# notu97/GS-SLAM-Analytica_Jacobian

Hardware: AMD Instinct MI355X
Metric: Gaussian-pixel interactions/sec (fwd+Jacobian), 640x480 (higher is better)
Workload: dtype f32; 1 GPU; cfg2: 50000 Gaussians (SH degree 3, 16 coeffs), 640x480; one step = one mapping window of 8 keyframes with distinct cameras: forward splat + analytical-Jacobian backward (dL/dmu, dL/dSigma->conic, per-Gaussian grads summed over the window, one dL/dtau per keyframe)

## Files before the change

### gs-slam-analytica_jacobian_amd/csrc/gsaj_common.h

```cpp
#pragma once
#include <hip/hip_runtime.h>
#include <stddef.h>
#include <stdint.h>

#include "../../include/gsaj.h"

#define GSAJ_WAVE 64
#define TILE GSAJ_TILE
#define TILE_PIXELS (TILE * TILE)
#define PRE_BLOCK 256
#define GB_BLOCK 64
#define REC_F4 3
#define IGRAD_F 12


#include "workspace.h"
#define WS_MEMBER(field, type, count) type *field;
#define WS_TAKE(field, type, count) w->field = c.take<type>(count);
#define WS_SHIFT(field, type, count) w.field = gsaj_shift(w.field, off);

#define GEOM_WS_FIELDS(X)                                                                                                          \
  X(depths, float, P)                               \
  X(cov3D, float, P * 6)               \
  X(clamped, uint8_t, P * 3)                                                                                                       \
  X(tiles_touched, uint32_t, P)                                                                                                    \
  X(point_offsets, uint32_t, P)     \
  X(internal_radii, int, P)                                                                                                        \
  X(block_sums, uint32_t, nblk)                               \
  X(tau_partials, float, ((P + 31) / 32 + 1) * 8)    \
  X(splat, float4, P * 3)                     \
  X(splat16, float4, P * 2)        \
                                          \
  X(scat, uint2, P)                        \
                                                                                                           \
  X(gsum, float4, P * 3)               \
struct GeomWS { GEOM_WS_FIELDS(WS_MEMBER) };

static inline size_t geom_carve(Carver c, size_t P, GeomWS *w) {
  size_t nblk = (P + PRE_BLOCK - 1) / PRE_BLOCK;
  if (nblk == 0) nblk = 1;
  GEOM_WS_FIELDS(WS_TAKE)
  return c.used();
}

#define TILE_REP 1
#define LDS_TILES_MAX 8192
#define SORT_CAP 16384
#define N_COUNTERS 64
#define ERR_PREFILTERED 1u
#define ERR_INTERNAL 2u
#define ERR_CAPACITY 4u
#define ERR_TILE_LIST 8u

#define IMAGE_WS_HEAD(X)                                                                                                           \
  X(final_T, float, N)                                                                                                             \
  X(n_contrib, uint32_t, N)                                                                                                        \
  X(ranges, uint2, tiles)
#define IMAGE_WS_ZEROED(X)                                                                                                         \
  X(counters, uint32_t, N_COUNTERS)                                                                                                \
  X(tile_count, uint32_t, tiles * TILE_REP)                                                                                        \
  X(tile_cursor, uint32_t, tiles * TILE_REP)
#define IMAGE_WS_TAIL(X)                                                                                                           \
  X(tile_offset, uint32_t, tiles * TILE_REP + 1)                                    \
  X(sticky, uint32_t, 16)             \
                                                                                                \
  X(tile_order, uint32_t, tiles)
#define IMAGE_WS_FIELDS(X) IMAGE_WS_HEAD(X) IMAGE_WS_ZEROED(X) IMAGE_WS_TAIL(X)
struct ImageWS {
  IMAGE_WS_FIELDS(WS_MEMBER)
  size_t zero_bytes;
};

static inline size_t image_carve(Carver c, int W, int H, ImageWS *w) {
  const size_t N = (size_t)W * H;
  const size_t tiles = (size_t)((W + TILE - 1) / TILE) * ((H + TILE - 1) / TILE);
  IMAGE_WS_HEAD(WS_TAKE)
  const size_t z0 = c.used();
  IMAGE_WS_ZEROED(WS_TAKE)
  w->zero_bytes = c.used() - z0;
  IMAGE_WS_TAIL(WS_TAKE)
  return c.used();
}

#define BIN_WS_FIELDS(X)                                                                                                           \
  X(keys_unsorted, uint64_t, R)      \
  X(keys, uint64_t, R)              \
                                       \
                                                                                                    \
  X(point_list, uint32_t, R)           \
                                                                                                              \
  X(inst_grad, float4, R * REC_F4)                        \
  X(reached, uint8_t, R)            \
                                                          \
  X(taken, uint32_t, R)            \
                                    \
                                       \
struct BinWS { BIN_WS_FIELDS(WS_MEMBER) };

static inline size_t bin_carve(Carver c, size_t R, BinWS *w) {
  if (R == 0) R = 1;
  BIN_WS_FIELDS(WS_TAKE)
  return c.used();
}

struct ViewStrides {
  size_t geom, image, bin;
};
#ifdef __HIPCC__
#include <type_traits>
template <typename T>
__device__ __forceinline__ T *gsaj_shift(T *p, size_t bytes) {
  typedef typename std::conditional<std::is_const<T>::value, const char, char>::type byte_t;
  return reinterpret_cast<T *>(reinterpret_cast<byte_t *>(p) + bytes);
}
__device__ __forceinline__ GeomWS geom_view(GeomWS w, size_t off) {
  GEOM_WS_FIELDS(WS_SHIFT)
  return w;
}
__device__ __forceinline__ ImageWS image_view(ImageWS w, size_t off) {
  IMAGE_WS_FIELDS(WS_SHIFT)
  return w;
}
#endif

struct Carved { GeomWS g; BinWS b; ImageWS im; ViewStrides vs; };

void gsaj_set_error(const char *fmt, ...);
#define GSAJ_HIP_CHECK(expr)                                                          \
  do {                                                                                \
    hipError_t _e = (expr);                                                           \
    if (_e != hipSuccess) {                                                           \
      gsaj_set_error("%s failed: %s (%s:%d)", #expr, hipGetErrorString(_e), __FILE__, __LINE__); \
      return GSAJ_ERR_HIP;                                                            \
    }                                                                                 \
  } while (0)

enum GsajStage {
  ST_PREPROCESS = 0, ST_SCAN, ST_EMIT_KEYS, ST_SORT, ST_RANGES_RECORDS, ST_RENDER_FWD, ST_RENDER_BWD, ST_GAUSSIAN_BWD,
  ST_TAU_FINALIZE, ST_DENSE_BWD, ST_DENSE_REDUCE, ST_SCATTER, ST_TILE_SORT, ST_GATHER_SUMS, ST_COUNT
};
void gsaj_prof_mark(int stage, int is_stop, hipStream_t s);
struct GsajProfScope {
  int stage;
  hipStream_t s;
  GsajProfScope(int st, hipStream_t stream) : stage(st), s(stream) { gsaj_prof_mark(stage, 0, s); }
  ~GsajProfScope() { gsaj_prof_mark(stage, 1, s); }
};

struct FwdParams {
  int P, D, M, W, H;
  const float *means3D, *shs, *colors_precomp, *opacities, *scales, *rotations, *cov3D_precomp;
  const float *viewmatrix, *projmatrix, *campos;
  float scale_modifier, tanfovx, tanfovy, focal_x, focal_y;
  int prefiltered;
  int grid_x, grid_y;
  int capacity;
  int sort_cap;
  int bpw;
  int views;
};

struct PreprocessPlan {
  int bpw;
  int workgroups;
  bool hist_lds;
};
struct ScatterPlan {
  int gpt;
  int workgroups;
  bool counters_lds;
};
PreprocessPlan plan_preprocess(int P, int views, int grid_x, int grid_y);
ScatterPlan plan_scatter(int P, int views, int grid_x, int grid_y);

#define LDS_DEFAULT_LIMIT 65536
struct LdsRequest {
  size_t dynamic_bytes, static_bytes, limit_bytes;
  int variant;
};
constexpr size_t lds_static_round(size_t bytes) { return (bytes + 3) / 4 * 4; }
LdsRequest lds_preprocess(const PreprocessPlan &pl, int grid_x, int grid_y, bool sh16);
LdsRequest lds_frame_scan(const PreprocessPlan &pl, int grid_x, int grid_y);
LdsRequest lds_scatter(const ScatterPlan &pl, int grid_x, int grid_y);
struct SortPlan {
  int launches;
  int keys[2];
  int pass[2];
  LdsRequest lds[2];
};
SortPlan plan_tile_sort(int sort_cap);
LdsRequest lds_gaussian_bwd(int M, bool has_shs);
bool lds_stereo_winner(int W, int D, LdsRequest *out);

int launch_preprocess(const FwdParams &p, int *radii, int *n_touched, const GeomWS &g, const ImageWS &im, ViewStrides vs,
                      hipStream_t s);
int launch_tile_binning(int P, int sort_cap, int rec16, int grid_x, int grid_y, const GeomWS &g, const BinWS &b, const ImageWS &im,
                        int views, ViewStrides vs, hipStream_t s);
struct FusedLoss;
int launch_render_forward(int P, int W, int H, int grid_x, int grid_y, const float *bg, const GeomWS &g, const BinWS &b,
                          const ImageWS &im, float *out_color, float *out_depth, float *out_opacity, int *n_touched, int views,
                          ViewStrides vs, hipStream_t s, const FusedLoss *fl = nullptr);
int gsaj_fwd_loss_slots(int W, int H);
int launch_loss_finalize(const FusedLoss &fl, int nslots, int W, int H, const uint32_t *aborted, float *out_scalars, hipStream_t s,
                         int views = 1, size_t abort_stride = 0, float *out_dexposure = nullptr);
int launch_render_backward(int R, int W, int H, int grid_x, int grid_y, const float *bg, const GeomWS &g, const BinWS &b,
                           const ImageWS &im, const float *dL_dpix, const float *dL_dpix_depth, int views, ViewStrides vs,
                           hipStream_t s, const FusedLoss *fl = nullptr);
int launch_export_taken(int W, int H, int grid_x, int grid_y, const BinWS &b, const ImageWS &im, uint32_t *out, hipStream_t s);
struct BwdParams {
  int P, D, M, W, H;
  const float *means3D, *shs, *scales, *rotations, *cov3Ds;
  const float *viewmatrix, *projmatrix, *projmatrix_raw, *campos;
  float scale_modifier, tanfovx, tanfovy, focal_x, focal_y;
  int grid_x, grid_y;
  const int *radii;
  float *dL_dmean2D, *dL_dconic, *dL_dopacity, *dL_dcolor, *dL_ddepth, *dL_dmean3D, *dL_dcov3D, *dL_dsh, *dL_dscale,
      *dL_drot, *dL_dtau, *dL_dtau_sum;
};
int launch_gaussian_backward(const BwdParams &p, const GeomWS &g, const BinWS &b, const ImageWS &im, hipStream_t s);
int launch_gather_sums(int P, int K, const int *radii, const GeomWS &g, const BinWS &b, const ImageWS &im, ViewStrides vs, hipStream_t s);
int launch_gaussian_backward_batch(const BwdParams &p, int K, const GeomWS &g, const BinWS &b, const ImageWS &im, ViewStrides vs,
                                   int accumulate, int gather, hipStream_t s);
size_t gsaj_jac_rows_bytes(int P);
int gsaj_jac_slots(int W, int H);
int launch_splat_jac(const BwdParams &p, int K, const GeomWS &g, const ImageWS &im, float *rows, ViewStrides vs, size_t rows_stride,
                     hipStream_t s);
struct JacOut {
  float *jac;
  float *color, *depth;
  const float *seed_c, *seed_d;
  const float *curv_c, *curv_d;
  float *partials;
  float delta;
};
int launch_render_jac(const BwdParams &p, int K, const float *bg, const Carved &c, const float *rows, size_t rows_stride, const JacOut &jo,
                      const FusedLoss *fl, int joint, hipStream_t s);
int launch_gn_reduce(const float *partials, int n, const ImageWS &im, float *H_out, float *g_out, hipStream_t s);
int launch_mark_visible(int P, const float *means3D, const float *viewmatrix, uint8_t *present, hipStream_t s);
void launch_exclusive_scan_u32(int n, uint32_t *v, hipStream_t s);
int launch_select_rank_f32(int W, int H, const float *values, uint32_t rank, uint32_t *out_key, void *seed_ws, hipStream_t s);
hipError_t launch_stereo_paths(int D, int W, int H, int first_col, int P1, int P2, int paths, const uint16_t *C, uint32_t *S, hipStream_t s);

#ifdef __HIPCC__
__device__ __forceinline__ float3 xform4x3(const float *m, float3 p) {
  return make_float3(m[0] * p.x + m[4] * p.y + m[8] * p.z + m[12], m[1] * p.x + m[5] * p.y + m[9] * p.z + m[13],
                     m[2] * p.x + m[6] * p.y + m[10] * p.z + m[14]);
}
__device__ __forceinline__ float4 xform4x4(const float *m, float3 p) {
  return make_float4(m[0] * p.x + m[4] * p.y + m[8] * p.z + m[12], m[1] * p.x + m[5] * p.y + m[9] * p.z + m[13],
                     m[2] * p.x + m[6] * p.y + m[10] * p.z + m[14], m[3] * p.x + m[7] * p.y + m[11] * p.z + m[15]);
}
__device__ __forceinline__ float ndc2pix(float v, int S) { return (float)((((double)v + 1.0) * (double)S - 1.0) * 0.5); }

__device__ __forceinline__ uint32_t gsaj_tile_band(const uint32_t *__restrict__ sticky) {
  const uint32_t band = sticky[1];
  return sticky[2] == ~band ? band : 0u;
}
__device__ __forceinline__ void tile_rect(float px, float py, int r, int gx, int gy, uint32_t band, int &x0, int &y0, int &x1,
                                          int &y1) {
  const int ylo = band ? (int)(band & 0xffffu) : 0, yhi = band ? min(gy, (int)(band >> 16)) : gy;
  x0 = min(gx, max(0, (int)((px - (float)r) / (float)TILE)));
  y0 = min(yhi, max(ylo, (int)((py - (float)r) / (float)TILE)));
  x1 = min(gx, max(0, (int)((px + (float)r + (float)(TILE - 1)) / (float)TILE)));
  y1 = min(yhi, max(ylo, (int)((py + (float)r + (float)(TILE - 1)) / (float)TILE)));
}
#define GSAJ_LOG2E 1.4426950408889634f
__device__ __forceinline__ float3 gsaj_prescale_conic(float a, float b, float c) {
  return make_float3((-0.5f * GSAJ_LOG2E) * a, -GSAJ_LOG2E * b, (-0.5f * GSAJ_LOG2E) * c);
}
__device__ __forceinline__ float gsaj_power2(float dx, float dy, float kx, float ky, float kz) {
  const float t = ky * dy;
  const float u = kz * dy;
  return __builtin_fmaf(dx, __builtin_fmaf(kx, dx, t), u * dy);
}
__device__ __forceinline__ bool quadrant_relevant(float mx, float my, float a, float b, float c, float o, float X0,
                                                  float Y0) {
  const float dxl = mx - (X0 + 7.0f), dxh = mx - X0;
  const float dyl = my - (Y0 + 7.0f), dyh = my - Y0;
  const bool pd = a > 0.f && c > 0.f && (a * c - b * b) > 0.f;
  const bool inside = dxl <= 0.f && dxh >= 0.f && dyl <= 0.f && dyh >= 0.f;
  const float ic = __builtin_amdgcn_rcpf(c), ia = __builtin_amdgcn_rcpf(a);
  float q = 3.0e38f;
  {
    const float y0 = fminf(fmaxf(-b * dxl * ic, dyl), dyh);
    q = fminf(q, a * dxl * dxl + 2.f * b * dxl * y0 + c * y0 * y0);
    const float y1 = fminf(fmaxf(-b * dxh * ic, dyl), dyh);
    q = fminf(q, a * dxh * dxh + 2.f * b * dxh * y1 + c * y1 * y1);
    const float x0 = fminf(fmaxf(-b * dyl * ia, dxl), dxh);
    q = fminf(q, a * x0 * x0 + 2.f * b * x0 * dyl + c * dyl * dyl);
    const float x1 = fminf(fmaxf(-b * dyh * ia, dxl), dxh);
    q = fminf(q, a * x1 * x1 + 2.f * b * x1 * dyh + c * dyh * dyh);
  }
  const float qs = fmaxf(q * 0.999f - 1.0e-3f, 0.f);
  const bool reach = o * __expf(-0.5f * qs) >= (0.99f / 255.0f);
  return !pd || inside || reach;
}
__device__ __forceinline__ float3 cross3(float3 a, float3 b) {
  return make_float3(a.y * b.z - a.z * b.y, a.z * b.x - a.x * b.z, a.x * b.y - a.y * b.x);
}
#endif

#define REC16_F4 2
#ifdef __HIPCC__
#include <hip/hip_fp16.h>
__device__ __forceinline__ uint32_t gsaj_pack_h2(float a, float b) {
  const __half2 h = __floats2half2_rn(a, b);
  return *reinterpret_cast<const uint32_t *>(&h);
}
__device__ __forceinline__ float2 gsaj_unpack_h2(uint32_t u) { return __half22float2(*reinterpret_cast<const __half2 *>(&u)); }
__device__ __forceinline__ void gsaj_load_row(const float4 *__restrict__ splat, const float4 *__restrict__ splat16, uint32_t id,
                                              bool rec16, float4 &q0, float4 &q1, float4 &q2) {
  if (!rec16) {
    const float4 *s = splat + (size_t)id * REC_F4;
    const float4 r0 = s[0], r1 = s[1], r2 = s[2];
    q0 = make_float4(r0.x, r0.y, r2.w, r0.w);
    q1 = r1;
    q2 = make_float4(r2.x, r2.y, r2.z, r0.z);
    return;
  }
  const float4 *s = splat16 + (size_t)id * REC16_F4;
  const float4 p0 = s[0], p1 = s[1];
  const float2 ab = gsaj_unpack_h2(__float_as_uint(p1.x)), co = gsaj_unpack_h2(__float_as_uint(p1.y));
  const float2 rg = gsaj_unpack_h2(__float_as_uint(p1.z)), bz = gsaj_unpack_h2(__float_as_uint(p1.w));
  q0 = p0;
  q1 = make_float4(ab.x, ab.y, co.x, co.y);
  q2 = make_float4(rg.x, rg.y, bz.x, 0.f);
}
#endif

#ifdef __HIPCC__
__device__ __forceinline__ float4 gsaj_load_f4_unaligned(const void *src) {
  typedef float f4u __attribute__((ext_vector_type(4), aligned(4)));
  const f4u v = *reinterpret_cast<const __attribute__((address_space(1))) f4u *>((unsigned long long)src);
  return make_float4(v.x, v.y, v.z, v.w);
}
__device__ __forceinline__ uint32_t gsaj_load_u32_global(const uint32_t *src) {
  return *reinterpret_cast<const __attribute__((address_space(1))) uint32_t *>((unsigned long long)src);
}
__device__ __forceinline__ uint2 gsaj_load_u64_device(const uint2 *src) {
  const unsigned long long v = __hip_atomic_load(reinterpret_cast<const __attribute__((address_space(1))) unsigned long long *>((unsigned long long)src),
                                                 __ATOMIC_RELAXED, __HIP_MEMORY_SCOPE_AGENT);
  return make_uint2((uint32_t)v, (uint32_t)(v >> 32));
}
#endif

#ifdef GSAJ_BLOCK_TRACE
#define GSAJ_TRACE_MAX 65536
#define GSAJ_TRACE_DEFINE(NAME)                                                                               \
  __device__ unsigned long long g_trace_##NAME[4 * GSAJ_TRACE_MAX];                                           \
  extern "C" int gsaj_trace_read_##NAME(unsigned long long *host, int nwaves) {                               \
    return (int)hipMemcpyFromSymbol(host, HIP_SYMBOL(g_trace_##NAME), sizeof(unsigned long long) * 4 * nwaves); \
  }
#define GSAJ_TRACE_BEGIN(NAME)                                                                                \
  {                                                                                                           \
    const unsigned tw_ = (blockIdx.y * gridDim.x + blockIdx.x) * (blockDim.x >> 6) + (threadIdx.x >> 6);      \
    if ((threadIdx.x & 63) == 0 && tw_ < GSAJ_TRACE_MAX) {                                                    \
      g_trace_##NAME[4 * tw_ + 0] = wall_clock64();                                                           \
      g_trace_##NAME[4 * tw_ + 2] = __builtin_amdgcn_s_getreg((4) | (0 << 6) | (31 << 11));                   \
      g_trace_##NAME[4 * tw_ + 3] = __builtin_amdgcn_s_getreg((20) | (0 << 6) | (31 << 11));                  \
    }                                                                                                         \
  }
#define GSAJ_TRACE_END(NAME)                                                                                  \
  {                                                                                                           \
    const unsigned tw_ = (blockIdx.y * gridDim.x + blockIdx.x) * (blockDim.x >> 6) + (threadIdx.x >> 6);      \
    if ((threadIdx.x & 63) == 0 && tw_ < GSAJ_TRACE_MAX) g_trace_##NAME[4 * tw_ + 1] = wall_clock64();        \
  }
#else
#define GSAJ_TRACE_DEFINE(NAME)
#define GSAJ_TRACE_BEGIN(NAME)
#define GSAJ_TRACE_END(NAME)
#endif
```

### gs-slam-analytica_jacobian_amd/csrc/render_fwd.hip

```cpp
#include "gsaj_common.h"
#include "loss_terms.h"
#include "wave_reduce.h"

#define FWD_CHUNK 64
#define FWD_PAD 8
#define FWD_PAIR_F4 6
typedef float v2f __attribute__((ext_vector_type(2)));

#ifndef GSAJ_FWD_THREADS
#define GSAJ_FWD_THREADS 64
#endif
#define FWD_WAVES (GSAJ_FWD_THREADS / 64)

GSAJ_TRACE_DEFINE(fwd)

template <bool LOSS>
__global__ __launch_bounds__(GSAJ_FWD_THREADS) __attribute__((amdgpu_waves_per_eu(6, 8))) void k_render_fwd(int W, int H, int gx, int tiles, int P, ImageWS im,
                                                    const float4 *__restrict__ splat, const float4 *__restrict__ splat16,
                                                    const float *__restrict__ bg,
                                                    float *__restrict__ out_color, float *__restrict__ out_depth,
                                                    float *__restrict__ out_opacity, int *__restrict__ n_touched,
                                                    const uint32_t *__restrict__ point_list, uint32_t *__restrict__ taken,
                                                    ViewStrides vs, FusedLoss fl) {
  {
    const size_t view = blockIdx.y, HWv = (size_t)H * W;
    im = image_view(im, view * vs.image);
    splat = gsaj_shift(splat, view * vs.geom);
    splat16 = gsaj_shift(splat16, view * vs.geom);
    point_list = gsaj_shift(point_list, view * vs.bin);
    taken = gsaj_shift(taken, view * vs.bin);
    out_color += view * 3 * HWv;
    out_depth += view * HWv;
    out_opacity += view * HWv;
    n_touched += view * (size_t)P;
    if (LOSS) fused_loss_view(fl, view, HWv, gridDim.x);
  }
  const uint2 *__restrict__ ranges = im.ranges;
  float *__restrict__ final_T = im.final_T;
  uint32_t *__restrict__ n_contrib = im.n_contrib;
  uint32_t *__restrict__ counters = im.counters;
  __shared__ float4 rec_all[FWD_WAVES * ((FWD_CHUNK + FWD_PAD) / 2) * FWD_PAIR_F4];
  if (counters[4]) return;
  GSAJ_TRACE_BEGIN(fwd)
  const int tid = threadIdx.x, lane = tid & 63;
#if FWD_WAVES == 1
  const int wave = ((int)blockIdx.x >> 3) & 3;
  const int rank = ((int)blockIdx.x >> 5) * 8 + ((int)blockIdx.x & 7);
  if (rank >= tiles) {
    if (LOSS && lane == 0) reinterpret_cast<float4 *>(fl.partials)[blockIdx.x] = make_float4(0.f, 0.f, 0.f, 0.f);
    return;
  }
  const int tile = (int)min(im.tile_order[rank], (uint32_t)(tiles - 1));
  float4 *rec = rec_all;
#else
  const int wave = tid >> 6;
  const int tile = (int)min(im.tile_order[blockIdx.x], (uint32_t)(tiles - 1));
  float4 *rec = rec_all + wave * ((FWD_CHUNK + FWD_PAD) / 2) * FWD_PAIR_F4;
#endif
  const int ty = tile / gx, tx = tile - ty * gx;
  const int px = tx * TILE + (wave & 1) * 8 + (lane & 7);
  const int py = ty * TILE + (wave >> 1) * 8 + (lane >> 3);
  const bool inside = px < W && py < H;
  const float pxf = (float)px, pyf = (float)py;
  const float qx0 = (float)(tx * TILE + (wave & 1) * 8), qy0 = (float)(ty * TILE + (wave >> 1) * 8);
  const uint2 range = ranges[tile];

  unsigned long long done_m = __builtin_amdgcn_ballot_w64(!inside);
  float T = 1.0f;
  uint32_t last = 0;
  bool counting = true;

  auto sel = [](unsigned long long m, float a, float b) -> float {
    float r;
    asm("v_cndmask_b32_e64 %0, %1, %2, %3" : "=v"(r) : "v"(b), "v"(a), "s"(m));
    return r;
  };
  auto sel0 = [](unsigned long long m, float a) -> float {
    float r;
    asm("v_cndmask_b32_e64 %0, 0, %1, %2" : "=v"(r) : "v"(a), "s"(m));
    return r;
  };
  v2f Crg = {0.f, 0.f}, Cbd = {0.f, 0.f};
  const v2f px2 = {pxf, pxf}, py2 = {pyf, pyf};
  auto composite2 = [&](const float4 p0, const float4 p1, const float4 p2, const float4 cA, const float4 cB, const float2 pos,
                        float &T_afterA, unsigned long long &okA, unsigned long long &okB) {
    const v2f dx = v2f{p0.x, p0.y} - px2, dy = v2f{p0.z, p0.w} - py2;
    const v2f t = v2f{p1.z, p1.w} * dy;
    const v2f u = v2f{p2.x, p2.y} * dy;
    const v2f pw = __builtin_elementwise_fma(dx, __builtin_elementwise_fma(v2f{p1.x, p1.y}, dx, t), u * dy);
    const v2f oe = v2f{p2.z, p2.w} * v2f{__builtin_amdgcn_exp2f(pw.x), __builtin_amdgcn_exp2f(pw.y)};
    {
      const float alpha0 = fminf(0.99f, oe.x);
      const float tA = __builtin_fmaf(-alpha0, T, T);
      const unsigned long long pre = __builtin_amdgcn_ballot_w64(pw.x <= 0.0f) & __builtin_amdgcn_ballot_w64(alpha0 >= (1.0f / 255.0f)) & ~done_m;
      const unsigned long long sat = pre & __builtin_amdgcn_ballot_w64(tA < 0.0001f);
      done_m |= sat;
      okA = pre & ~sat;
      const float w = sel0(okA, alpha0 * T);
      const v2f w2 = {w, w};
      Crg = __builtin_elementwise_fma(v2f{cA.x, cA.y}, w2, Crg);
      Cbd = __builtin_elementwise_fma(v2f{cA.z, cA.w}, w2, Cbd);
      T = sel(okA, tA, T);
      last = __float_as_uint(sel(okA, pos.x, __uint_as_float(last)));
      T_afterA = T;
    }
    {
      const float alpha0 = fminf(0.99f, oe.y);
      const float tB = __builtin_fmaf(-alpha0, T, T);
      const unsigned long long pre = __builtin_amdgcn_ballot_w64(pw.y <= 0.0f) & __builtin_amdgcn_ballot_w64(alpha0 >= (1.0f / 255.0f)) & ~done_m;
      const unsigned long long sat = pre & __builtin_amdgcn_ballot_w64(tB < 0.0001f);
      done_m |= sat;
      okB = pre & ~sat;
      const float w = sel0(okB, alpha0 * T);
      const v2f w2 = {w, w};
      Crg = __builtin_elementwise_fma(v2f{cB.x, cB.y}, w2, Crg);
      Cbd = __builtin_elementwise_fma(v2f{cB.z, cB.w}, w2, Cbd);
      T = sel(okB, tB, T);
      last = __float_as_uint(sel(okB, pos.y, __uint_as_float(last)));
    }
  };

  if (~done_m != 0ull && range.x < range.y) {
    float4 q0, q1, q2;
    uint32_t id_cur = 0u, id_nxt = 0u;
    const bool rec16 = counters[7] != 0u;
    auto fetch_id = [&](uint32_t base) {
      if (base + (uint32_t)lane < range.y) id_nxt = point_list[base + lane];
    };
    auto fetch_row = [&](uint32_t base) {
      id_cur = id_nxt;
      if (base + (uint32_t)lane < range.y) gsaj_load_row(splat, splat16, id_nxt, rec16, q0, q1, q2);
    };
    float *recf = reinterpret_cast<float *>(rec);
    for (int i = lane; i < ((FWD_CHUNK + FWD_PAD) / 2) * FWD_PAIR_F4; i += 64) rec[i] = make_float4(0.f, 0.f, 0.f, 0.f);
    auto put = [&](int s, float x, float y, float kx, float ky, float kz, float o, float4 c, uint32_t pos, uint32_t id) {
      const int h = s & 1, pb = (s >> 1) * FWD_PAIR_F4;
      float *f = recf + pb * 4 + h;
      f[0] = x; f[2] = y; f[4] = kx; f[6] = ky; f[8] = kz; f[10] = o;
      rec[pb + 3 + h] = c;
      f[20] = __uint_as_float(pos); f[22] = __uint_as_float(id);
    };
    fetch_id(range.x);
    fetch_row(range.x);
    fetch_id(range.x + FWD_CHUNK);
    for (uint32_t base = range.x; base < range.y; base += FWD_CHUNK) {
      const int m = min((uint32_t)FWD_CHUNK, range.y - base);
      bool rel = false;
      const uint32_t id_here = id_cur;
      if (lane < m) rel = quadrant_relevant(q0.x, q0.y, q1.x, q1.y, q1.z, q1.w, qx0, qy0);
      const unsigned long long todo = __builtin_amdgcn_ballot_w64(rel);
      const int nrel = __popcll(todo);
      __builtin_amdgcn_wave_barrier();
      if (rel) {
        const int slot = __builtin_amdgcn_mbcnt_hi((uint32_t)(todo >> 32), __builtin_amdgcn_mbcnt_lo((uint32_t)todo, 0u));
        const float3 k = gsaj_prescale_conic(q1.x, q1.y, q1.z);
        put(slot, q0.x, q0.y, k.x, k.y, k.z, q1.w, make_float4(q2.x, q2.y, q2.z, q0.z), base - range.x + (uint32_t)lane + 1u, id_here);
      }
      if (lane < FWD_PAD) recf[((nrel + lane) >> 1) * FWD_PAIR_F4 * 4 + 10 + ((nrel + lane) & 1)] = 0.f;
      fetch_row(base + FWD_CHUNK);
      fetch_id(base + 2 * FWD_CHUNK);
      __builtin_amdgcn_fence(__ATOMIC_RELEASE, "wavefront");
      __builtin_amdgcn_wave_barrier();
      __builtin_amdgcn_fence(__ATOMIC_ACQUIRE, "wavefront");
      uint32_t cnt4 = 0u;
      bool wave_done = false;
      const float2 *rec2 = reinterpret_cast<const float2 *>(rec);
      float4 a0 = rec[0], a1 = rec[1], a2 = rec[2], a3 = rec[3], a4 = rec[4];
      float2 a5 = rec2[10];
      for (int i = 0; i < nrel; i += 4) {
        const int pb = (i >> 1) * FWD_PAIR_F4;
        const float4 c0 = rec[pb + 6], c1 = rec[pb + 7], c2 = rec[pb + 8], c3 = rec[pb + 9], c4 = rec[pb + 10];
        const float2 c5 = rec2[(pb + 11) * 2];
        uint32_t pack;
        {
          float Ta;
          unsigned long long okA, okB;
          composite2(a0, a1, a2, a3, a4, a5, Ta, okA, okB);
          pack = (okA != 0ull ? 0x80u : 0u) | (okB != 0ull ? 0x8000u : 0u);
          if (counting) {
            const unsigned long long hB = __builtin_amdgcn_ballot_w64(T > 0.5f);
            const uint32_t nA = (uint32_t)__popcll(__builtin_amdgcn_ballot_w64(Ta > 0.5f) & okA);
            const uint32_t nB = (uint32_t)__popcll(hB & okB);
            pack |= nA | (nB << 8);
            counting = hB != 0ull;
          }
        }
        asm volatile("" : "+v"(T), "+v"(last), "+v"(Crg), "+v"(Cbd) : : "memory");
        a0 = rec[pb + 12], a1 = rec[pb + 13], a2 = rec[pb + 14], a3 = rec[pb + 15], a4 = rec[pb + 16];
        a5 = rec2[(pb + 17) * 2];
        {
          float Tc;
          unsigned long long okC, okD;
          composite2(c0, c1, c2, c3, c4, c5, Tc, okC, okD);
          pack |= (okC != 0ull ? 0x800000u : 0u) | (okD != 0ull ? 0x80000000u : 0u);
          if (counting) {
            const unsigned long long hD = __builtin_amdgcn_ballot_w64(T > 0.5f);
            const uint32_t nC = (uint32_t)__popcll(__builtin_amdgcn_ballot_w64(Tc > 0.5f) & okC);
            const uint32_t nD = (uint32_t)__popcll(hD & okD);
            pack |= (nC << 16) | (nD << 24);
            counting = hD != 0ull;
          }
        }
        cnt4 = ((lane >> 2) == (i >> 2)) ? pack : cnt4;
        if (~done_m == 0ull) {
          wave_done = true;
          break;
        }
      }
      const uint32_t mine = (cnt4 >> (8 * (lane & 3))) & 0xffu;
      const int cnt = (int)(mine & 0x7fu);
      if (lane < nrel && cnt > 0) {
        const uint32_t id = __float_as_uint(recf[(lane >> 1) * FWD_PAIR_F4 * 4 + 22 + (lane & 1)]);
        atomicAdd(&n_touched[id], cnt);
      }
      const int slot = __builtin_amdgcn_mbcnt_hi((uint32_t)(todo >> 32), __builtin_amdgcn_mbcnt_lo((uint32_t)todo, 0u));
      const uint32_t took = (uint32_t)__shfl((int)mine, slot) >> 7;
      if (lane < m) {
        reinterpret_cast<uint8_t *>(taken + base)[(uint32_t)(lane * 4 + wave)] = rel ? (uint8_t)took : (uint8_t)0;
      }
      __builtin_amdgcn_wave_barrier();
      if (wave_done) break;
    }
  }

  const float Cr = Crg.x, Cg = Crg.y, Cb = Cbd.x, Dp = Cbd.y;
  int lane_e = lane;
  asm volatile("" : "+v"(lane_e));
  const int px_e = tx * TILE + (wave & 1) * 8 + (lane_e & 7), py_e = ty * TILE + (wave >> 1) * 8 + (lane_e >> 3);
  if (inside) {
    const size_t pid = (size_t)py_e * W + px_e;
    const size_t HW = (size_t)H * W;
    final_T[pid] = T;
    n_contrib[pid] = last;
    out_color[pid] = Cr + T * bg[0];
    out_color[HW + pid] = Cg + T * bg[1];
    out_color[2 * HW + pid] = Cb + T * bg[2];
    out_depth[pid] = Dp;
    out_opacity[pid] = 1.f - T;
  }
  if (LOSS) {
    float s4[4] = {0.f, 0.f, 0.f, 0.f};
    if (inside) {
      const size_t pid = (size_t)py_e * W + px_e, HW = (size_t)H * W;
      const LossConsts L = loss_consts(fl.flags, fl.alpha, fl.rgb_thr, fl.exp_a, fl.exp_b, HW, 1.f);
      const bool mask = fl.grad_mask ? fl.grad_mask[pid] != 0 : true;
      const float gd = L.mono ? 0.f : fl.gt_depth[pid];
      const LossPixel o = loss_pixel(L, fl.gt_color[pid], fl.gt_color[HW + pid], fl.gt_color[2 * HW + pid], Cr + T * bg[0], Cg + T * bg[1],
                                     Cb + T * bg[2], 1.f - T, mask, gd, Dp);
      s4[0] = o.s_rgb; s4[1] = o.s_d; s4[2] = o.s_a; s4[3] = o.s_b;
    }
#pragma unroll
    for (int c = 0; c < 4; c++) s4[c] = wave_sum(s4[c]);
    if (lane == 0) reinterpret_cast<float4 *>(fl.partials)[blockIdx.x] = make_float4(s4[0], s4[1], s4[2], s4[3]);
  }
  GSAJ_TRACE_END(fwd)
}

int gsaj_fwd_loss_slots(int W, int H) {
  const int tiles = ((W + TILE - 1) / TILE) * ((H + TILE - 1) / TILE);
  return FWD_WAVES == 1 ? ((tiles + 7) / 8) * 32 : tiles;
}

int launch_render_forward(int P, int W, int H, int grid_x, int grid_y, const float *bg, const GeomWS &g, const BinWS &b,
                          const ImageWS &im, float *out_color, float *out_depth, float *out_opacity, int *n_touched, int views,
                          ViewStrides vs, hipStream_t s, const FusedLoss *fl) {
  static_assert(FWD_WAVES == 1, "the loss-fused epilogue writes one partial per wave-sized workgroup");
  {
    GsajProfScope ps(ST_RENDER_FWD, s);
    const int tiles = grid_x * grid_y;
    const unsigned nblk = FWD_WAVES == 1 ? (unsigned)((tiles + 7) / 8) * 32u : (unsigned)tiles;
    if (fl)
      hipLaunchKernelGGL(k_render_fwd<true>, dim3(nblk, views), dim3(GSAJ_FWD_THREADS), 0, s, W, H, grid_x, tiles, P, im, g.splat, g.splat16, bg,
                         out_color, out_depth, out_opacity, n_touched, b.point_list, b.taken, vs, *fl);
    else
      hipLaunchKernelGGL(k_render_fwd<false>, dim3(nblk, views), dim3(GSAJ_FWD_THREADS), 0, s, W, H, grid_x, tiles, P, im, g.splat, g.splat16,
                         bg, out_color, out_depth, out_opacity, n_touched, b.point_list, b.taken, vs, FusedLoss{});
  }
  GSAJ_HIP_CHECK(hipGetLastError());
  return GSAJ_OK;
}
```

Before: 731.8 billion interactions/s.

## Carry leftover relevant Gaussians across chunks to keep forward quad steps full

The forward render loop walks compacted Gaussians in groups of four. Previously each chunk's tail group was padded with zero-opacity sentinels. Now, except on the last chunk, up to three leftover entries are carried into the next chunk's staging area, so every quad step processes real Gaussians. Because carried entries can be settled in a later chunk, the per-entry taken/n_touched bookkeeping now uses each entry's stored position. This adds an extra wave barrier and a small LDS copy per chunk, and handles a second pack word when more than 64 entries are staged.

```diff
diff --git a/gs-slam-analytica_jacobian_amd/csrc/gsaj_common.h b/gs-slam-analytica_jacobian_amd/csrc/gsaj_common.h
--- a/gs-slam-analytica_jacobian_amd/csrc/gsaj_common.h
+++ b/gs-slam-analytica_jacobian_amd/csrc/gsaj_common.h
@@ -94,7 +94,7 @@
                                                           \
   X(taken, uint32_t, R)            \
                                     \
-                                       \
+                                   \
 struct BinWS { BIN_WS_FIELDS(WS_MEMBER) };
 
 static inline size_t bin_carve(Carver c, size_t R, BinWS *w) {
diff --git a/gs-slam-analytica_jacobian_amd/csrc/render_fwd.hip b/gs-slam-analytica_jacobian_amd/csrc/render_fwd.hip
--- a/gs-slam-analytica_jacobian_amd/csrc/render_fwd.hip
+++ b/gs-slam-analytica_jacobian_amd/csrc/render_fwd.hip
@@ -3,8 +3,12 @@
 #include "wave_reduce.h"
 
 #define FWD_CHUNK 64
+#define FWD_CARRY 3
+#define FWD_SENTINELS 3
 #define FWD_PAD 8
 #define FWD_PAIR_F4 6
+static_assert(FWD_CARRY + FWD_CHUNK + FWD_SENTINELS + 2 <= FWD_CHUNK + FWD_PAD && (FWD_CARRY + FWD_CHUNK + FWD_SENTINELS) % 2 == 0,
+              "the staging area is too small for a full chunk behind a full carry");
 typedef float v2f __attribute__((ext_vector_type(2)));
 
 #ifndef GSAJ_FWD_THREADS
@@ -69,6 +73,9 @@
   float T = 1.0f;
   uint32_t last = 0;
   bool counting = true;
+#ifdef GSAJ_BLOCK_TRACE
+  uint32_t tr_steps = 0u, tr_surv = 0u, tr_sent = 0u;
+#endif
 
   auto sel = [](unsigned long long m, float a, float b) -> float {
     float r;
@@ -143,31 +150,40 @@
     fetch_id(range.x);
     fetch_row(range.x);
     fetch_id(range.x + FWD_CHUNK);
+    uint8_t *__restrict__ taken_q = reinterpret_cast<uint8_t *>(taken + range.x) + wave;
+    uint32_t carry = 0u;
     for (uint32_t base = range.x; base < range.y; base += FWD_CHUNK) {
       const int m = min((uint32_t)FWD_CHUNK, range.y - base);
       bool rel = false;
       const uint32_t id_here = id_cur;
       if (lane < m) rel = quadrant_relevant(q0.x, q0.y, q1.x, q1.y, q1.z, q1.w, qx0, qy0);
       const unsigned long long todo = __builtin_amdgcn_ballot_w64(rel);
-      const int nrel = __popcll(todo);
+      const int n = (int)carry + __popcll(todo);
+      const int nwalk = base + FWD_CHUNK < range.y ? (n & ~3) : n;
       __builtin_amdgcn_wave_barrier();
       if (rel) {
-        const int slot = __builtin_amdgcn_mbcnt_hi((uint32_t)(todo >> 32), __builtin_amdgcn_mbcnt_lo((uint32_t)todo, 0u));
+        const int slot = __builtin_amdgcn_mbcnt_hi((uint32_t)(todo >> 32), __builtin_amdgcn_mbcnt_lo((uint32_t)todo, carry));
         const float3 k = gsaj_prescale_conic(q1.x, q1.y, q1.z);
         put(slot, q0.x, q0.y, k.x, k.y, k.z, q1.w, make_float4(q2.x, q2.y, q2.z, q0.z), base - range.x + (uint32_t)lane + 1u, id_here);
       }
-      if (lane < FWD_PAD) recf[((nrel + lane) >> 1) * FWD_PAIR_F4 * 4 + 10 + ((nrel + lane) & 1)] = 0.f;
+      if (lane < FWD_SENTINELS) recf[((n + lane) >> 1) * FWD_PAIR_F4 * 4 + 10 + ((n + lane) & 1)] = 0.f;
       fetch_row(base + FWD_CHUNK);
       fetch_id(base + 2 * FWD_CHUNK);
       __builtin_amdgcn_fence(__ATOMIC_RELEASE, "wavefront");
       __builtin_amdgcn_wave_barrier();
       __builtin_amdgcn_fence(__ATOMIC_ACQUIRE, "wavefront");
-      uint32_t cnt4 = 0u;
+      uint32_t cnt4 = 0u, pack_hi = 0u;
       bool wave_done = false;
       const float2 *rec2 = reinterpret_cast<const float2 *>(rec);
       float4 a0 = rec[0], a1 = rec[1], a2 = rec[2], a3 = rec[3], a4 = rec[4];
       float2 a5 = rec2[10];
-      for (int i = 0; i < nrel; i += 4) {
+#ifdef GSAJ_BLOCK_TRACE
+      const uint32_t tr_steps0 = tr_steps;
+#endif
+      for (int i = 0; i < nwalk; i += 4) {
+#ifdef GSAJ_BLOCK_TRACE
+        tr_steps++;
+#endif
         const int pb = (i >> 1) * FWD_PAIR_F4;
         const float4 c0 = rec[pb + 6], c1 = rec[pb + 7], c2 = rec[pb + 8], c3 = rec[pb + 9], c4 = rec[pb + 10];
         const float2 c5 = rec2[(pb + 11) * 2];
@@ -202,24 +218,44 @@
           }
         }
         cnt4 = ((lane >> 2) == (i >> 2)) ? pack : cnt4;
+        if (i == FWD_CHUNK) pack_hi = pack;
         if (~done_m == 0ull) {
           wave_done = true;
           break;
         }
       }
-      const uint32_t mine = (cnt4 >> (8 * (lane & 3))) & 0xffu;
-      const int cnt = (int)(mine & 0x7fu);
-      if (lane < nrel && cnt > 0) {
-        const uint32_t id = __float_as_uint(recf[(lane >> 1) * FWD_PAIR_F4 * 4 + 22 + (lane & 1)]);
-        atomicAdd(&n_touched[id], cnt);
+      const int nst = wave_done ? n : nwalk;
+#ifdef GSAJ_BLOCK_TRACE
+      {
+        const uint32_t walked = 4u * (tr_steps - tr_steps0), surv = min(walked, (uint32_t)n);
+        tr_surv += surv;
+        tr_sent += walked - surv;
       }
-      const int slot = __builtin_amdgcn_mbcnt_hi((uint32_t)(todo >> 32), __builtin_amdgcn_mbcnt_lo((uint32_t)todo, 0u));
-      const uint32_t took = (uint32_t)__shfl((int)mine, slot) >> 7;
-      if (lane < m) {
-        reinterpret_cast<uint8_t *>(taken + base)[(uint32_t)(lane * 4 + wave)] = rel ? (uint8_t)took : (uint8_t)0;
+#endif
+      auto settle = [&](int s, uint32_t word4) {
+        const uint32_t mine = (word4 >> (8 * (s & 3))) & 0xffu;
+        const float *f = recf + (s >> 1) * FWD_PAIR_F4 * 4 + (s & 1);
+        const int cnt = (int)(mine & 0x7fu);
+        if (cnt > 0) atomicAdd(&n_touched[__float_as_uint(f[22])], cnt);
+        taken_q[(__float_as_uint(f[20]) - 1u) * 4u] = (uint8_t)(mine >> 7);
+      };
+      if (lane < nst) settle(lane, cnt4);
+      if (nst > 64 && lane < nst - 64) settle(64 + lane, pack_hi);
+      if (lane < m && !rel) taken_q[(base - range.x + (uint32_t)lane) * 4u] = (uint8_t)0;
+      if (wave_done) break;
+      carry = (uint32_t)(n - nwalk);
+      __builtin_amdgcn_fence(__ATOMIC_RELEASE, "wavefront");
+      __builtin_amdgcn_wave_barrier();
+      __builtin_amdgcn_fence(__ATOMIC_ACQUIRE, "wavefront");
+      if (carry != 0u && nwalk != 0) {
+        if (lane < 2 * FWD_PAIR_F4) {
+          const float4 v = rec[(nwalk >> 1) * FWD_PAIR_F4 + lane];
+          rec[lane] = v;
+        }
+        __builtin_amdgcn_fence(__ATOMIC_RELEASE, "wavefront");
+        __builtin_amdgcn_wave_barrier();
+        __builtin_amdgcn_fence(__ATOMIC_ACQUIRE, "wavefront");
       }
-      __builtin_amdgcn_wave_barrier();
-      if (wave_done) break;
     }
   }
 
@@ -254,6 +290,15 @@
     if (lane == 0) reinterpret_cast<float4 *>(fl.partials)[blockIdx.x] = make_float4(s4[0], s4[1], s4[2], s4[3]);
   }
   GSAJ_TRACE_END(fwd)
+#ifdef GSAJ_BLOCK_TRACE
+  {
+    const unsigned tw_ = blockIdx.y * gridDim.x + blockIdx.x;
+    if (lane == 0 && tw_ < GSAJ_TRACE_MAX) {
+      g_trace_fwd[4 * tw_ + 2] = (g_trace_fwd[4 * tw_ + 2] & 0xffffffffull) | ((unsigned long long)tr_steps << 32);
+      g_trace_fwd[4 * tw_ + 3] = (g_trace_fwd[4 * tw_ + 3] & 0xffffffffull) | ((unsigned long long)tr_surv << 32) | ((unsigned long long)tr_sent << 48);
+    }
+  }
+#endif
 }
 
 int gsaj_fwd_loss_slots(int W, int H) {
```

Result: no change. 732.0 billion interactions/s, median of 2 (+0.0%).
